# Visual-Behavior/detr-tensorflow

Hardware: AMD Instinct MI355X
Metric: images/sec training step, DETR-R50 800x1333 bs=8/GPU (higher is better)
Workload: dtype bf16

## Files before the change

detr-tensorflow_amd/csrc/optim.hip:

```cpp
#include "common.h"

namespace detr {

__global__ __launch_bounds__(256) void sumsq_segments_kernel(const float *__restrict__ g,
                                                             const int *__restrict__ chunk_tensor,
                                                             const long long *__restrict__ chunk_start,
                                                             const long long *__restrict__ seg_end, int chunk,
                                                             float *__restrict__ sumsq) {
    __shared__ float red[4];
    const int c = blockIdx.x;
    const int t = chunk_tensor[c];
    const long long s0 = chunk_start[c];
    long long s1 = s0 + chunk;
    if (s1 > seg_end[t]) s1 = seg_end[t];
    float acc = 0.f;
    for (long long i = s0 + threadIdx.x; i < s1; i += blockDim.x) {
        const float v = g[i];
        acc += v * v;
    }
    acc = wave_sum(acc);
    if ((threadIdx.x & 63) == 0) red[threadIdx.x >> 6] = acc;
    __syncthreads();
    if (threadIdx.x == 0) sumsq[c] = (red[0] + red[1]) + (red[2] + red[3]);
}

__device__ __forceinline__ float clip_factor(float nrm, float clip) { return nrm > clip ? clip / nrm : (nrm == nrm ? 1.0f : nrm); }

__global__ __launch_bounds__(256) void clip_adam_kernel(float *__restrict__ param, const float *__restrict__ g,
                                                        float *__restrict__ m, float *__restrict__ v,
                                                        const int *__restrict__ chunk_tensor,
                                                        const long long *__restrict__ chunk_start,
                                                        const long long *__restrict__ seg_end,
                                                        const int *__restrict__ tensor_group,
                                                        const float *__restrict__ sumsq,
                                                        const float *__restrict__ hyper, int chunk, int n_chunks) {
    const int c = blockIdx.x;
    const int t = chunk_tensor[c];
    const long long s0 = chunk_start[c];
    long long s1 = s0 + chunk;
    if (s1 > seg_end[t]) s1 = seg_end[t];
    const int grp = tensor_group[t];
    if (grp < 0) return;
    const float lr_t = hyper[grp];
    const float clip = hyper[3], b1 = hyper[4], b2 = hyper[5], eps = hyper[6];
    float cs = 1.0f;
    if (clip > 0.f) {
        __shared__ int s_lo, s_hi;
        __shared__ float s_red[4];
        if (threadIdx.x == 0) {
            int a = 0, b = c;
            while (a < b) { const int mid = (a + b) >> 1; if (chunk_tensor[mid] < t) a = mid + 1; else b = mid; }
            s_lo = a;
            a = c; b = n_chunks;
            while (a < b) { const int mid = (a + b) >> 1; if (chunk_tensor[mid] <= t) a = mid + 1; else b = mid; }
            s_hi = a;
        }
        __syncthreads();
        float acc = 0.f;
        for (int k = s_lo + (int)threadIdx.x; k < s_hi; k += blockDim.x) acc += sumsq[k];
        acc = wave_sum(acc);
        if ((threadIdx.x & 63) == 0) s_red[threadIdx.x >> 6] = acc;
        __syncthreads();
        const float nrm = sqrtf((s_red[0] + s_red[1]) + (s_red[2] + s_red[3]));
        cs = clip_factor(nrm, clip);
    }
    for (long long i = s0 + threadIdx.x; i < s1; i += blockDim.x) {
        const float gi = g[i] * cs;
        const float mi = b1 * m[i] + (1.0f - b1) * gi;
        const float vi = b2 * v[i] + (1.0f - b2) * gi * gi;
        m[i] = mi;
        v[i] = vi;
        param[i] = param[i] - lr_t * mi / (sqrtf(vi) + eps);
    }
}

__global__ void set_floats8_kernel(float *dst, float v0, float v1, float v2, float v3, float v4, float v5, float v6,
                                   float v7) {
    if (threadIdx.x == 0 && blockIdx.x == 0) {
        dst[0] = v0; dst[1] = v1; dst[2] = v2; dst[3] = v3; dst[4] = v4; dst[5] = v5; dst[6] = v6; dst[7] = v7;
    }
}

struct Floats16 { float v[16]; };

__global__ void set_floats16_kernel(float *dst, Floats16 f) {
    if (blockIdx.x == 0 && threadIdx.x < 16) dst[threadIdx.x] = f.v[threadIdx.x];
}

__global__ __launch_bounds__(256) void global_clip_scale_kernel(const float *__restrict__ sumsq,
                                                                const int *__restrict__ chunk_tensor,
                                                                const int *__restrict__ tensor_group,
                                                                const float *__restrict__ hyper, int n_chunks,
                                                                float *__restrict__ scale) {
    __shared__ float red[4];
    float acc = 0.f;
    for (int k = threadIdx.x; k < n_chunks; k += 256) {
        const int grp = tensor_group[chunk_tensor[k]];
        if (grp >= 0 && hyper[11 + grp] != 0.f) acc += sumsq[k];
    }
    acc = wave_sum(acc);
    if ((threadIdx.x & 63) == 0) red[threadIdx.x >> 6] = acc;
// ... 252 lines not shown
```

detr-tensorflow_amd/csrc/rowops.hip:

```cpp
#include "common.h"

namespace detr {

constexpr int LN_MAXV = 4;

__device__ __forceinline__ unsigned ln_pk_bf16(float a, float b) {
    typedef __bf16 bf16x2_t __attribute__((ext_vector_type(2)));
    bf16x2_t r;
    r[0] = (__bf16)a;
    r[1] = (__bf16)b;
    return __builtin_bit_cast(unsigned, r);
}

__global__ __launch_bounds__(256) void layernorm_fwd_kernel(const float *__restrict__ x, const float *__restrict__ gamma,
                                                            const float *__restrict__ beta, float *__restrict__ y,
                                                            float *__restrict__ mean, float *__restrict__ rstd,
                                                            int rows, int C, float eps, const float *__restrict__ add,
                                                            int add_rows, float *__restrict__ y2, unsigned short *__restrict__ y16) {
    const int lane = threadIdx.x & 63;
    const int wpb = blockDim.x >> 6;
    const int nv = C >> 2;
    for (int row = blockIdx.x * wpb + (threadIdx.x >> 6); row < rows; row += gridDim.x * wpb) {
        const float4 *xr = reinterpret_cast<const float4 *>(x + (long long)row * C);
        float4 v[LN_MAXV];
// ... 319 lines not shown
                           C, d->dgamma, d->dbeta);
        DETR_LAUNCH_CHECK("layernorm bwd finish");
    }
    return 0;
}

namespace detr {
typedef __bf16 bf16x2_t __attribute__((ext_vector_type(2)));
__device__ __forceinline__ unsigned pk2_bf16(float a, float b) {
    bf16x2_t r;
    r[0] = (__bf16)a;
    r[1] = (__bf16)b;
    return __builtin_bit_cast(unsigned, r);
}
__global__ void cvt_bf16_kernel(const float4 *__restrict__ x, uint2 *__restrict__ out, long long n4) {
    for (long long i = blockIdx.x * (long long)blockDim.x + threadIdx.x; i < n4; i += (long long)gridDim.x * blockDim.x) {
        const float4 v = x[i];
        out[i] = make_uint2(pk2_bf16(v.x, v.y), pk2_bf16(v.z, v.w));
    }
}
__global__ void scale_cols_bf16_kernel(const float4 *__restrict__ w, const float4 *__restrict__ scale, uint2 *__restrict__ out,
                                       long long n4, int c4) {
    for (long long i = blockIdx.x * (long long)blockDim.x + threadIdx.x; i < n4; i += (long long)gridDim.x * blockDim.x) {
        const float4 v = w[i], sc = scale[i % c4];
        out[i] = make_uint2(pk2_bf16(v.x * sc.x, v.y * sc.y), pk2_bf16(v.z * sc.z, v.w * sc.w));
    }
}

static_assert(sizeof(detr_scale_entry) == 40, "detr_scale_entry layout changed: update Engine._refold_group");

__global__ void scale_cols_bf16_group_kernel(const detr_scale_entry *__restrict__ tab) {
    const detr_scale_entry e = tab[blockIdx.y];
    const float4 *w = reinterpret_cast<const float4 *>(e.w), *scale = reinterpret_cast<const float4 *>(e.scale);
    uint2 *out = reinterpret_cast<uint2 *>(e.out);
    for (long long i = blockIdx.x * (long long)blockDim.x + threadIdx.x; i < e.n4; i += (long long)gridDim.x * blockDim.x) {
        const float4 v = w[i], sc = scale[i % e.c4];
        out[i] = make_uint2(pk2_bf16(v.x * sc.x, v.y * sc.y), pk2_bf16(v.z * sc.z, v.w * sc.w));
    }
}
}

extern "C" int detr_hip_scale_cols_bf16_group(const detr_scale_entry *table, int32_t n, void *stream) {
    DETR_REQUIRE(table && n > 0 && n <= 65535, "scale_cols_bf16_group: bad args");
    hipLaunchKernelGGL(scale_cols_bf16_group_kernel, dim3(64, (unsigned)n), dim3(256), 0, (hipStream_t)stream, table);
    DETR_LAUNCH_CHECK("scale_cols_bf16_group");
    return 0;
}

extern "C" int detr_hip_cvt_bf16(const float *x, uint16_t *out, int64_t n, void *stream) {
    DETR_REQUIRE(x && out && n > 0 && n % 4 == 0 && aligned16(x) && ((uintptr_t)out % 8 == 0), "cvt_bf16: bad args");
    const long long n4 = n / 4;
    long long grid = (n4 + 255) / 256;
    if (grid > 8192) grid = 8192;
    hipLaunchKernelGGL(cvt_bf16_kernel, dim3((unsigned)grid), dim3(256), 0, (hipStream_t)stream, (const float4 *)x, (uint2 *)out, n4);
    DETR_LAUNCH_CHECK("cvt_bf16");
    return 0;
}

extern "C" int detr_hip_scale_cols_bf16(const float *w, const float *scale, uint16_t *out, int64_t rows, int32_t cols,
                                        void *stream) {
    DETR_REQUIRE(w && scale && out && rows > 0 && cols > 0 && cols % 4 == 0, "scale_cols_bf16: bad args");
    DETR_REQUIRE(aligned16(w) && aligned16(scale) && ((uintptr_t)out % 8 == 0), "scale_cols_bf16: alignment");
    const long long n4 = rows * (long long)(cols / 4);
    long long grid = (n4 + 255) / 256;
    if (grid > 8192) grid = 8192;
    hipLaunchKernelGGL(scale_cols_bf16_kernel, dim3((unsigned)grid), dim3(256), 0, (hipStream_t)stream, (const float4 *)w,
                       (const float4 *)scale, (uint2 *)out, n4, cols / 4);
    DETR_LAUNCH_CHECK("scale_cols_bf16");
    return 0;
}

extern "C" int detr_hip_colsum_f32(const float *x, float *out, int64_t rows, int32_t cols, int64_t ld, float alpha,
                                   void *stream) {
    DETR_REQUIRE(x && out && rows > 0 && cols > 0, "colsum: bad args");
    int rpb = 64;
    while ((rows + rpb - 1) / rpb > 2048) rpb *= 2;
    dim3 grid((unsigned)cdiv(cols, 256), (unsigned)((rows + rpb - 1) / rpb));
    hipLaunchKernelGGL(colsum_kernel, grid, dim3(256), 0, (hipStream_t)stream, x, out, (long long)rows, cols,
                       (long long)ld, alpha, rpb);
    DETR_LAUNCH_CHECK("colsum");
    return 0;
}

__global__ __launch_bounds__(256) void colsum_partial_kernel(const float *__restrict__ x, float *__restrict__ part, long long rows, int cols,
                                                             long long ld, int rows_per_block) {
    const int c = blockIdx.x * 256 + threadIdx.x;
    if (c >= cols) return;
    const long long r0 = (long long)blockIdx.y * rows_per_block;
    const long long r1 = (r0 + rows_per_block < rows) ? r0 + rows_per_block : rows;
    float s0 = 0.f, s1 = 0.f;
    long long r = r0;
    for (; r + 1 < r1; r += 2) {
        s0 += x[r * ld + c];
        s1 += x[(r + 1) * ld + c];
    }
    if (r < r1) s0 += x[r * ld + c];
    part[(long long)blockIdx.y * cols + c] = s0 + s1;
}
__global__ __launch_bounds__(256) void colsum_finish_kernel(const float *__restrict__ part, float *__restrict__ out, int chunks, int cols, float alpha) {
    const int c = blockIdx.x * 256 + threadIdx.x;
    if (c >= cols) return;
    float s = 0.f;
    for (int k = 0; k < chunks; ++k) s += part[(long long)k * cols + c];
    out[c] += alpha * s;
}
static int colsum_det_rpb(int64_t rows) {
    int rpb = 64;
    while ((rows + rpb - 1) / rpb > 256) rpb *= 2;
    return rpb;
}
extern "C" int64_t detr_hip_colsum_det_scratch_floats(int64_t rows, int32_t cols) {
    if (rows <= 0 || cols <= 0) return -1;
    const int rpb = colsum_det_rpb(rows);
    return ((rows + rpb - 1) / rpb) * (int64_t)cols;
}
extern "C" int detr_hip_colsum_det_f32(const float *x, float *out, int64_t rows, int32_t cols, int64_t ld, float alpha, float *scratch,
                                       int64_t scratch_floats, void *stream) {
    DETR_REQUIRE(x && out && scratch && rows > 0 && cols > 0, "colsum_det: bad args");
    const int rpb = colsum_det_rpb(rows);
    const int chunks = (int)((rows + rpb - 1) / rpb);
    DETR_REQUIRE(scratch_floats >= (int64_t)chunks * cols, "colsum_det: scratch holds %lld floats, %lld needed", (long long)scratch_floats,
                 (long long)chunks * cols);
    hipLaunchKernelGGL(colsum_partial_kernel, dim3((unsigned)cdiv(cols, 256), (unsigned)chunks), dim3(256), 0, (hipStream_t)stream, x, scratch,
                       (long long)rows, cols, (long long)ld, rpb);
    hipLaunchKernelGGL(colsum_finish_kernel, dim3((unsigned)cdiv(cols, 256)), dim3(256), 0, (hipStream_t)stream, scratch, out, chunks, cols, alpha);
    DETR_LAUNCH_CHECK("colsum_det");
    return 0;
}

extern "C" int detr_hip_add_bcast_f32(const float *x, const float *p, float *out, int64_t n, int64_t period,
                                      void *stream) {
    DETR_REQUIRE(x && p && out && n > 0 && period > 0, "add_bcast: bad args");
    DETR_REQUIRE(n % 4 == 0 && period % 4 == 0 && aligned16(x) && aligned16(p) && aligned16(out), "add_bcast: alignment");
    hipLaunchKernelGGL(add_bcast_kernel, dim3(capped_grid(n / 4, 256, 8192)), dim3(256), 0, (hipStream_t)stream, (const float4 *)x,
                       (const float4 *)p, (float4 *)out, (long long)(n / 4), (long long)(period / 4));
    DETR_LAUNCH_CHECK("add_bcast");
    return 0;
}

extern "C" int detr_hip_add_f32(const float *a, const float *b, float *out, int64_t n, void *stream) {
    DETR_REQUIRE(a && b && out && n > 0, "add: bad args");
    hipLaunchKernelGGL(add_kernel, dim3(capped_grid(n, 256, 8192)), dim3(256), 0, (hipStream_t)stream, a, b, out, (long long)n);
    DETR_LAUNCH_CHECK("add");
    return 0;
}

extern "C" int detr_hip_sigmoid_bwd_f32(const float *dy, const float *y, float *dz, int64_t n, void *stream) {
    DETR_REQUIRE(dy && y && dz && n > 0, "sigmoid_bwd: bad args");
    hipLaunchKernelGGL(sigmoid_bwd_kernel, dim3(capped_grid(n, 256, 8192)), dim3(256), 0, (hipStream_t)stream, dy, y, dz,
                       (long long)n);
    DETR_LAUNCH_CHECK("sigmoid_bwd");
    return 0;
}

extern "C" int detr_hip_dropout_f32(const float *x, float *out, int64_t n, float p, uint32_t site, const uint32_t *step,
                                    void *stream) {
    DETR_REQUIRE(x && out && n > 0 && p >= 0.0f && p < 1.0f, "dropout: bad args");
    hipLaunchKernelGGL(dropout_kernel, dim3(capped_grid(n, 256, 8192)), dim3(256), 0, (hipStream_t)stream, x, out, (long long)n,
                       1.0f / (1.0f - p), drop_thresh16(p), site, step);
    DETR_LAUNCH_CHECK("dropout");
    return 0;
}

namespace detr {
__global__ __launch_bounds__(256) void multi_copy_kernel(const detr_copy_entry *__restrict__ table) {
    const detr_copy_entry e = table[blockIdx.y];
    const uint4 *src = reinterpret_cast<const uint4 *>(e.src);
    uint4 *dst = reinterpret_cast<uint4 *>(e.dst);
    for (long long i = blockIdx.x * (long long)blockDim.x + threadIdx.x; i < e.n16; i += (long long)gridDim.x * blockDim.x) {
        if (e.mode == 0) {
            dst[i] = src[i];
        } else {
            const float4 a = reinterpret_cast<const float4 *>(src)[i];
            float4 b = reinterpret_cast<float4 *>(dst)[i];
            b.x += a.x; b.y += a.y; b.z += a.z; b.w += a.w;
            reinterpret_cast<float4 *>(dst)[i] = b;
        }
    }
}
__global__ void set_u32x8_kernel(uint32_t *dst, uint32_t v0, uint32_t v1, uint32_t v2, uint32_t v3, uint32_t v4, uint32_t v5,
                                 uint32_t v6, uint32_t v7) {
    if (threadIdx.x == 0) { dst[0] = v0; dst[1] = v1; dst[2] = v2; dst[3] = v3; dst[4] = v4; dst[5] = v5; dst[6] = v6; dst[7] = v7; }
}
}

namespace detr {
// ... 98 lines not shown
```

detr-tensorflow_amd/csrc/setloss.hip:

```cpp
#include "common.h"
#include <limits.h>
#include <cmath>
#include <type_traits>

namespace detr {

struct SetLossArgs {
    int levels, B, Q, C, R;
    const float *logits; long long sL_l, sL_b, sL_q;
    const float *boxes;  long long sB_l, sB_b, sB_q;
    const float *t_bbox; const long long *t_class;
    int background_class;
};

struct FixedCriterion {
    static constexpr float cost_class = 1.0f, cost_bbox = 5.0f, cost_giou = 2.0f;
    static constexpr float w_label = 1.0f, w_bbox = 5.0f, w_giou = 2.0f;
    static constexpr float eos = 0.1f;
    static constexpr bool weighted = false;
    __device__ __forceinline__ float class_weight(int, int) const { return 1.0f; }
    __device__ __forceinline__ float weight_sum(const float *s) const { return eos * s[3] + s[4]; }
    __device__ __forceinline__ float box_count(float npos) const { return npos; }
};

// ... 154 lines not shown

constexpr int SL_QCHUNK = 8;

template <class Crit, class Cls>
__global__ __launch_bounds__(256) void match_cost_kernel(SetLossArgs a, Crit crit, Cls clsterm, float *__restrict__ cost) {
    __shared__ typename Cls::Row s_row[SL_QCHUNK];
    __shared__ float s_t[SL_MAXR][4];
    __shared__ int s_cls[SL_MAXR];
    const int p = blockIdx.x;
    const int lv = p / a.B, b = p % a.B;
    const int n = header_n(a.t_bbox, b, a.R);
    const int ldc = a.R - 1;
    if (n == 0) return;
    const float *lg = a.logits + lv * a.sL_l + b * a.sL_b;
    const float *bx = a.boxes + lv * a.sB_l + b * a.sB_b;
    const int lane = threadIdx.x & 63, wave = threadIdx.x >> 6;
    for (int j = threadIdx.x; j < n; j += blockDim.x) {
        const float *t = a.t_bbox + ((long long)b * a.R + 1 + j) * 4;
        s_t[j][0] = t[0]; s_t[j][1] = t[1]; s_t[j][2] = t[2]; s_t[j][3] = t[3];
        s_cls[j] = (int)a.t_class[(long long)b * a.R + 1 + j];
    }
    const int q0 = blockIdx.y * SL_QCHUNK, q1 = min(a.Q, q0 + SL_QCHUNK);
    for (int q = q0 + wave; q < q1; q += 4) {
        const typename Cls::Row r = clsterm.row_stats(lg + q * a.sL_q, a.C, lane);
        if (lane == 0) s_row[q - q0] = r;
    }
    __syncthreads();
    float *out = cost + (long long)p * a.Q * ldc;
    for (int idx = threadIdx.x; idx < (q1 - q0) * n; idx += blockDim.x) {
        const int ql = idx / n, j = idx - ql * n;
        const int q = q0 + ql;
        const float *pb = bx + q * a.sB_q;
        const float pcx = pb[0], pcy = pb[1], pw = pb[2], ph = pb[3];
        const float tcx = s_t[j][0], tcy = s_t[j][1], tw = s_t[j][2], th = s_t[j][3];
        const int cls = s_cls[j];
        const float cost_class = (cls >= 0 && cls < a.C) ? clsterm.cost(s_row[ql], lg[q * a.sL_q + cls]) : 0.0f;
        const float cost_bbox = fabsf(pcx - tcx) + fabsf(pcy - tcy) + fabsf(pw - tw) + fabsf(ph - th);
        const float cost_giou = -giou_of(to_xyxy(pcx, pcy, pw, ph), to_xyxy(tcx, tcy, tw, th));
        out[q * ldc + j] = crit.cost_bbox * cost_bbox + crit.cost_class * cost_class + crit.cost_giou * cost_giou;
    }
}

template <int CTRL, int ROW_MASK>
__device__ __forceinline__ double dpp_min_step(double x, int &tlo, int &thi) {
    tlo = __builtin_amdgcn_update_dpp(tlo, __double2loint(x), CTRL, ROW_MASK, 0xf, false);
    thi = __builtin_amdgcn_update_dpp(thi, __double2hiint(x), CTRL, ROW_MASK, 0xf, false);
    const double y = __hiloint2double(thi, tlo);
    double r;
    asm("v_min_f64 %0, %1, %2" : "=v"(r) : "v"(x), "v"(y));
    return r;
}
__device__ __forceinline__ double wave_min_f64_dpp(double x) {
    int tlo = __double2loint(x), thi = __double2hiint(x);
    x = dpp_min_step<0x111, 0xf>(x, tlo, thi);
    x = dpp_min_step<0x112, 0xf>(x, tlo, thi);
    x = dpp_min_step<0x114, 0xf>(x, tlo, thi);
    x = dpp_min_step<0x118, 0xf>(x, tlo, thi);
    x = dpp_min_step<0x142, 0xa>(x, tlo, thi);
    x = dpp_min_step<0x143, 0xc>(x, tlo, thi);
    const int lo = __builtin_amdgcn_readlane(__double2loint(x), 63);
    const int hi = __builtin_amdgcn_readlane(__double2hiint(x), 63);
    return __hiloint2double(hi, lo);
}

template <int S, int N>
struct AssignPick {
    static __device__ __forceinline__ void run(unsigned long long (&todo)[N], unsigned long long (&live)[N],
                                               const unsigned long long (&freecol)[N], const int (&row4col)[N], int &jstar,
                                               int &r4, bool &isfree) {
        if (S + 1 == N || todo[S]) {
            const int l = ((int)__ffsll((long long)todo[S]) - 1) & 63;
            const unsigned long long bit = 1ull << l;
            todo[S] &= ~bit;
            live[S] &= ~bit;
            isfree = (freecol[S] & bit) != 0ull;
            r4 = __builtin_amdgcn_readlane(row4col[S], l);
            jstar = 64 * S + l;
        } else {
            AssignPick<(S + 1 < N ? S + 1 : S), N>::run(todo, live, freecol, row4col, jstar, r4, isfree);
        }
    }
};

template <int MAXCPL, bool CD>
__global__ __launch_bounds__(64) void assign_kernel(const float *__restrict__ cost, int Q, int ldc,
                                                    const float *__restrict__ t_bbox, int B, int R,
                                                    int *__restrict__ tgt_for_pred, int *__restrict__ pred_for_tgt,
                                                    int *__restrict__ status) {
    using CT = typename std::conditional<CD, double, float>::type;
    extern __shared__ __attribute__((aligned(16))) char smem[];
    const int p = blockIdx.x, b = p % B, lane = threadIdx.x;
    const int nmax = (R + 1) & ~1;
    const int n = header_n(t_bbox, b, R);
    const int cpl = (Q + 63) >> 6;
    const int Qs = CD ? MAXCPL * 64 + 1 : cpl * 64 + 1;
    double *u0 = reinterpret_cast<double *>(smem);
    int *col4row = reinterpret_cast<int *>(u0 + nmax);
    CT *cT = reinterpret_cast<CT *>(col4row + nmax);
    double *u = CD ? reinterpret_cast<double *>(cT) + (Qs - 1) : u0;
    const int us = CD ? Qs : 1;

    for (int q = lane; q < Q; q += 64) tgt_for_pred[(long long)p * Q + q] = -1;
    for (int j = lane; j < ldc; j += 64) pred_for_tgt[(long long)p * ldc + j] = -1;
    if (lane == 0) status[p] = 0;
    if (n == 0) return;
    if (n > Q) {
        if (lane == 0) status[p] = 2;
        return;
    }
    const float *Cg = cost + (long long)p * Q * ldc;
    bool bad = false;
    for (int idx = lane; idx < Q * n; idx += 64) {
        const int q = idx / n, j = idx - q * n;
        const float c = Cg[q * ldc + j];
        cT[j * Qs + q] = (CT)c;
        bad |= !(c == c) || (c == -INFINITY);
    }
    if (Qs > Q)
        for (int idx = lane; idx < (Qs - Q) * n; idx += 64) cT[(idx / (Qs - Q)) * Qs + Q + idx % (Qs - Q)] = (CT)INFINITY;
    __syncthreads();
    for (int i = lane; i < n; i += 64) {
        u[i * us] = 0.0;
        col4row[i] = -1;
    }
    __syncthreads();
    if (__any(bad)) {
        if (lane == 0) status[p] = 1;
        return;
    }
    double v[MAXCPL], spc[MAXCPL];
    int path[MAXCPL], row4col[MAXCPL];
    unsigned long long exist[MAXCPL];
    unsigned long long freecol[MAXCPL];
#pragma unroll
    for (int s = 0; s < MAXCPL; ++s) {
        v[s] = 0.0;
        spc[s] = INFINITY;
        path[s] = -1;
        row4col[s] = -1;
        const int cnt = Q - 64 * s;
        exist[s] = cnt >= 64 ? ~0ull : (cnt <= 0 ? 0ull : ((1ull << cnt) - 1ull));
        freecol[s] = exist[s];
    }
    for (int i = 0; i < n; ++i) {
        const CT *crow = cT + i * Qs;
        double best = INFINITY;
        int bestj = INT_MAX;
#pragma unroll
        for (int s = 0; s < MAXCPL; ++s) {
            const int j = lane + 64 * s;
            if (s < cpl && j < Q) {
                const double c = (double)crow[j];
                if (c < best) { best = c; bestj = j; }
            }
        }
        const double gmin = wave_min_f64_dpp(best);
        if (!(gmin < (double)INFINITY)) continue;
        const unsigned long long mall = __ballot(best == gmin);
        const int ownl = __ffsll((long long)mall) - 1;
        const int jstar = __builtin_amdgcn_readlane(bestj, ownl);
        const int owns = jstar >> 6;
        int r4 = -1;
#pragma unroll
        for (int s = 0; s < MAXCPL; ++s)
            if (s == owns) r4 = row4col[s];
        r4 = __builtin_amdgcn_readlane(r4, ownl);
        if (lane == 0) u[i * us] = gmin;
        if (r4 == -1) {
#pragma unroll
            for (int s = 0; s < MAXCPL; ++s) {
                if (s == owns && lane == ownl) row4col[s] = i;
                if (s == owns) freecol[s] &= ~(1ull << ownl);
            }
            if (lane == 0) col4row[i] = jstar;
        }
    }
    __syncthreads();
    bool infeasible = false;
    for (int cur = 0; cur < n; ++cur) {
        if (col4row[cur] != -1) continue;
        double minVal = 0.0;
        int i = cur;
        int sink = -1;
        unsigned long long live[MAXCPL], todo[MAXCPL];
#pragma unroll
        for (int s = 0; s < MAXCPL; ++s) {
            spc[s] = INFINITY;
            live[s] = exist[s];
            todo[s] = 0ull;
        }
        while (true) {
            const double ui = u[i * us];
            const CT *crow = cT + i * Qs + lane;
            CT cf[MAXCPL];
#pragma unroll
            for (int s = 0; s < MAXCPL; ++s) cf[s] = crow[CD ? 64 * s : 64 * (s < cpl ? s : cpl - 1)];
            unsigned long long any_todo = 0ull;
#pragma unroll
            for (int s = 0; s < MAXCPL; ++s) {
                const double r = minVal + (double)cf[s] - ui - v[s];
                const unsigned long long um = __builtin_amdgcn_ballot_w64(r < spc[s]) & live[s];
                const bool upd = __builtin_amdgcn_inverse_ballot_w64(um);
// ... 434 lines not shown
```

detr-tensorflow_amd/detr_tf/engine.py:

```python
import math
import os
from ctypes import byref, c_float
from typing import NamedTuple, Optional

import numpy as np
import torch

from . import _hip as hip
from .params import ParamStore, RESNET50_BLOCKS, block_names, bn_conv_pairs, stem_names
from .streams import DropMasks, SideStream

D = 256
HEADS = 8
HD = 32
FF = 2048
BN_EPS = 1e-5
KERAS_BN_EPS = 1.001e-5
LN_EPS = 1e-5
DEFER_REDUCE = os.environ.get("DETR_HIP_DEFER_REDUCE", "1") != "0"
WGRAD_STREAM = os.environ.get("DETR_HIP_WGRAD_STREAM", "1") != "0"
BWD_FUSED = os.environ.get("DETR_HIP_BWD_FUSED", "1") != "0"
DROPMASK_AHEAD = int(os.environ.get("DETR_HIP_DROPMASK_AHEAD", "2") or 0)
QK_ALPHA = float(HD) ** -0.5 * 1.4426950408889634


def mix32(x):
    x &= 0xFFFFFFFF
    x ^= x >> 16
    x = (x * 0x7FEB352D) & 0xFFFFFFFF
    x ^= x >> 15
    x = (x * 0x846CA68B) & 0xFFFFFFFF
    x ^= x >> 16
    return x


def step_seed(base_seed, step_no, rank=0):
    return mix32(mix32((base_seed + 0x9E3779B9 * step_no) & 0xFFFFFFFF) ^ ((rank * 0x85EBCA6B) & 0xFFFFFFFF))


def position_embedding_sine_host(H, W, num_pos_features=128, temperature=10000.0, eps=1e-6):
    y = (np.arange(1, H + 1, dtype=np.float32) / np.float32(H + eps) * np.float32(2 * math.pi)).astype(np.float32)
    x = (np.arange(1, W + 1, dtype=np.float32) / np.float32(W + eps) * np.float32(2 * math.pi)).astype(np.float32)
    k = np.arange(num_pos_features, dtype=np.float32)
    dim_t = np.power(np.float32(temperature), (2 * np.floor(k / 2) / np.float32(num_pos_features)).astype(np.float32)).astype(np.float32)
    py = (y[:, None] / dim_t[None, :]).astype(np.float32)
    px = (x[:, None] / dim_t[None, :]).astype(np.float32)
    ey = np.empty_like(py)
    ex = np.empty_like(px)
    ey[:, 0::2], ey[:, 1::2] = np.sin(py[:, 0::2]), np.cos(py[:, 1::2])
    ex[:, 0::2], ex[:, 1::2] = np.sin(px[:, 0::2]), np.cos(px[:, 1::2])
    pos = np.concatenate([np.broadcast_to(ey[:, None, :], (H, W, num_pos_features)),
                          np.broadcast_to(ex[None, :, :], (H, W, num_pos_features))], axis=2)
    return np.ascontiguousarray(pos.reshape(H * W, 2 * num_pos_features), dtype=np.float32)


def position_embedding_sine_table(n_max, num_pos_features=128, temperature=10000.0, eps=1e-6):
    k = np.arange(num_pos_features, dtype=np.float32)
    dim_t = np.power(np.float32(temperature), (2 * np.floor(k / 2) / np.float32(num_pos_features)).astype(np.float32)).astype(np.float32)
    tab = np.zeros((n_max + 1, n_max + 1, num_pos_features), np.float32)
    c = np.arange(0, n_max + 1, dtype=np.float32)
    for n in range(n_max + 1):
        y = (c / np.float32(n + eps) * np.float32(2 * math.pi)).astype(np.float32)
        py = (y[:, None] / dim_t[None, :]).astype(np.float32)
        tab[n, :, 0::2], tab[n, :, 1::2] = np.sin(py[:, 0::2]), np.cos(py[:, 1::2])
    return tab


def downsample_mask_nearest(mask, Hf, Wf):
    mask = np.asarray(mask)
    H, W = mask.shape[1:]
    sy = np.minimum((np.arange(Hf) * H) // Hf, H - 1)
    sx = np.minimum((np.arange(Wf) * W) // Wf, W - 1)
    return mask[:, sy][:, :, sx]


def dilation_flags(replace_stride_with_dilation):
    if replace_stride_with_dilation is None:
        return (False, False, False)
    flags = tuple(bool(f) for f in replace_stride_with_dilation)
    if len(flags) != 3:
        raise ValueError(f"replace_stride_with_dilation: expected 3 flags (layer2, layer3, layer4), got {len(flags)}")
    return flags


def feature_size(H, W, replace_stride_with_dilation=None):
    for halves in (True, True) + tuple(not f for f in dilation_flags(replace_stride_with_dilation)):
        if halves:
            H, W = (H - 1) // 2 + 1, (W - 1) // 2 + 1
    return H, W


def backbone_stride(replace_stride_with_dilation=None):
    return 4 * 2 ** sum(1 for f in dilation_flags(replace_stride_with_dilation) if not f)


class Block(NamedTuple):
    p: str
    n: dict
    x: torch.Tensor
    xs: torch.Tensor
    x1: torch.Tensor
    y1: torch.Tensor
    y2: torch.Tensor
    out: torch.Tensor
    h: int
    w: int
    ho: int
    wo: int
    h1: int
    w1: int
    M1: int
    s2: int
    cin: int
    d1: int
    d2: int
    stride: int
    first: bool
    out_bits: Optional[torch.Tensor]
    dil: int


class DetrEngine:
    def __init__(self, device="cuda:0", blocks=RESNET50_BLOCKS, num_enc=6, num_dec=6, num_queries=100,
                 num_classes=92, nb_class=None, seed=0, tf_backbone=False, replace_stride_with_dilation=(False, False, False)):
        self.dilate = dilation_flags(replace_stride_with_dilation)
        if tf_backbone and any(self.dilate):
            raise ValueError("replace_stride_with_dilation needs the reference backbone: tf.keras.applications.ResNet50 "
                             "(tf_backbone=True) has no such option")
        hip.load()
        self.device = torch.device(device)
        hip.ensure_workspace(self.device)
        if DEFER_REDUCE:
            hip.ensure_defer_workspace(self.device)
        self.blocks = tuple(blocks)
        self.num_enc, self.num_dec, self.Q = num_enc, num_dec, num_queries
        self.nb_class = nb_class
        self.C = num_classes if nb_class is None else nb_class
        self.tf_backbone = bool(tf_backbone)
        self.bn_eps = KERAS_BN_EPS if self.tf_backbone else BN_EPS
        self.P = ParamStore(self.device, blocks, num_enc, num_dec, num_queries, num_classes, nb_class, seed, tf_backbone=tf_backbone)
        self._stem = stem_names(self.tf_backbone)
        self._pairs = bn_conv_pairs(self.blocks, self.tf_backbone)
        self._bufs = {}
        self._buf_gen = 0
        self._pos_cache = {}
        self._pos_tables = {}
        self.key_valid = None
        self._attn_sites = ()
        self.attn_maps = {}
        self._shape = None
        self._adt = torch.float32
        self._block_recs = []
        self._feat_meta = None
        self._fold_table = self._shift_table = None
        self.bn_scale, self.bn_shift = {}, {}
        self._weights_version, self._built = 0, {}
        self.P.on_change = self._params_changed
        self.fold_bn()
        self.compute = 0
        self.f32_split = False
        self.dropout_p = 0.1
        self.dropout_seed = 0x5EED
        self.dp_rank = 0
        self._step_no = 0
        self._drop = (0.0, 0)
        self._step_seed = 0
        self._seed_dev = torch.zeros(8, dtype=torch.int32, device=self.device)
        self._cross = {}
        self._graph_replay = False
        self.phase_events = None
        self.side = SideStream(self.device)
        self.masks = DropMasks(self, HEADS)

    @property
    def gemm_mode(self):
        return 1 if self.compute == 1 else (2 if self.f32_split else 0)

    def bump_weights_version(self):
        self._weights_version += 1

    def _stale(self, key):
        if self._built.get(key) == self._weights_version:
            return False
        self._built[key] = self._weights_version
        return True

    def seed_of_step(self, step_no):
        return step_seed(self.dropout_seed, step_no, self.dp_rank)

    def advance_dropout_step(self):
        self._step_no += 1
        self._step_seed = self.seed_of_step(self._step_no)
        self.masks.settle()
        hip.call("detr_hip_set_u32x8", self._seed_dev.data_ptr(), self._step_seed, self.seed_of_step(self._step_no + 1),
                 0, 0, 0, 0, 0, 0)
        self._drop = (float(self.dropout_p), self._step_seed)
        return self._step_seed

    def phase(self, name):
        if self.phase_events is not None:
            ev = torch.cuda.Event(enable_timing=True)
            ev.record()
            self.phase_events.append((name, ev))

    def buf(self, name, shape, dtype=torch.float32):
        key = name
        t = self._bufs.get(key)
        shape = tuple(int(s) for s in shape)
        if t is None or tuple(t.shape) != shape or t.dtype != dtype:
            if t is not None:
                self._buf_gen += 1
            t = torch.empty(shape, dtype=dtype, device=self.device)
            self._bufs[key] = t
        return t

    @property
    def buf_generation(self):
        return self._buf_gen + hip.WS_GENERATION

    def buffer_bytes(self):
        return sum(t.numel() * t.element_size() for t in self._bufs.values())

    def fold_bn(self):
        for p, c in self.P.bn.items():
            raw = self.P.bn_raw[p]
            sc = self.buf(f"bnscale:{p}", (c,))
            sh = self.buf(f"bnshift:{p}", (c,))
            hip.call("detr_hip_bn_fold_f32", raw[0].data_ptr(), raw[1].data_ptr(), raw[2].data_ptr(), raw[3].data_ptr(),
                     sc.data_ptr(), sh.data_ptr(), c, c_float(self.bn_eps))
            self.bn_scale[p] = sc
            self.bn_shift[p] = self.buf(f"bnshift_eff:{p}", (c,)) if self.tf_backbone else sh
        self.bump_weights_version()
        self._fold_table = None
        self._shift_table = None

    def _refresh_bias_shift(self):
        if self._shift_table is None:
            rows = []
            for bn_name, conv_name in self._pairs:
                c = self.P.bn[bn_name]
                rows.append([self.P.views[f"{conv_name}/bias"].data_ptr(), self.bn_scale[bn_name].data_ptr(),
                             self._bufs[f"bnshift:{bn_name}"].data_ptr(), self.bn_shift[bn_name].data_ptr(), c])
            self._shift_table = torch.tensor(rows, dtype=torch.int64).to(self.device)
        hip.call("detr_hip_fma_vec_group", self._shift_table.data_ptr(), self._shift_table.shape[0])

    def _params_changed(self):
        self.fold_bn()

    def load_params(self, params):
        return self.P.load_dict(params)

    def _w(self, name):
        if self.compute == 1 and self.P.views16 is not None:
            return self.P.views16[name]
        return self.P.views[name]

    def _refresh_shadow(self):
        flat16 = self.P.shadow16()
        hip.call("detr_hip_cvt_bf16", self.P.flat.data_ptr(), flat16.data_ptr(), self.P.flat.numel())
        self._refold_group()

    def _refold_group(self):
        if self._fold_table is None:
            rows = []
            for bn_name, conv in self._pairs[1:]:
                conv_name = f"{conv}/kernel"
                w = self.P.views[conv_name]
                co = w.shape[-1]
                ws16 = self.buf(f"ws16:{conv_name}", w.shape, torch.bfloat16)
                rows.append([w.data_ptr(), self.bn_scale[bn_name].data_ptr(), ws16.data_ptr(), w.numel() // 4, co // 4])
            self._fold_table = torch.tensor(rows, dtype=torch.int64).to(self.device)
            self._fold_keep = [self.bn_scale, self._bufs]
        hip.call("detr_hip_scale_cols_bf16_group", self._fold_table.data_ptr(), self._fold_table.shape[0])

    def _scaled_kernel(self, conv_name, bn_name):
        w = self.P.views[conv_name]
        co = w.shape[-1]
        if self.compute == 1 and conv_name != f"{self._stem['conv']}/kernel":
            return self.buf(f"ws16:{conv_name}", w.shape, torch.bfloat16)
        ws = self.buf(f"ws:{conv_name}", w.shape)
        if self._stale(f"ws:{conv_name}"):
            hip.call("detr_hip_scale_cols_f32", w.data_ptr(), self.bn_scale[bn_name].data_ptr(), ws.data_ptr(),
                     w.numel() // co, co)
        return ws

    def _conv1x1_fwd(self, x, M, cin, cout, conv_name, bn_name, out, residual=None, act=1, maskbits_out=None):
        ws = self._scaled_kernel(conv_name, bn_name)
        shift = self.bn_shift[bn_name]
        ldr = cout if residual is not None else 0
        hip.gemm(M, cout, cin, x, cin, 1, ws, cout, 0, out, cout, bias=shift, residual=residual, ldr=ldr, act=act,
                 maskbits_out=maskbits_out)

    @staticmethod
    def _wgrad(M_out, N_out, K_red, A, lda, Bm, ldb, C, ldc, scale=None, alpha=1.0, compute=None):
        args, kwargs = hip.wgrad_call(M_out, N_out, K_red, A, lda, Bm, ldb, C, ldc, scale=scale, alpha=alpha, compute=compute)
        hip.gemm(*args, **kwargs)

    def _a16(self, base):
        return (f"{base}16", torch.bfloat16) if self.compute == 1 else (base, torch.float32)

    def _colsum(self, x2d, out, alpha=1.0):
        rows, cols = x2d.shape
        n = int(hip.load().detr_hip_colsum_det_scratch_floats(rows, cols))
        scratch = self.buf(f"colsum:{rows}x{cols}", (n,))
        hip.call("detr_hip_colsum_det_f32", x2d.data_ptr(), out.data_ptr(), rows, cols, x2d.stride(0), c_float(alpha),
                 scratch.data_ptr(), n)

    def _ln_fwd(self, x, pfx, y, tag, add=None, y2=None, y16=None):
        rows = x.shape[0]
        mean = self.buf(f"{tag}:mean", (rows,))
        rstd = self.buf(f"{tag}:rstd", (rows,))
        hip.layernorm_fwd(x, self.P.views[f"{pfx}/gamma"], self.P.views[f"{pfx}/beta"], y, mean, rstd, LN_EPS, add=add, y2=y2,
                          y16=y16)

    def _ln_spec(self, rows, pfx, y, tag, add=None, y2=None, y16=None, ffn=False):
        if self.compute != 1 or ffn:
            return None
        return dict(gamma=self.P.views[f"{pfx}/gamma"], beta=self.P.views[f"{pfx}/beta"], y=y, mean=self.buf(f"{tag}:mean", (rows,)),
                    rstd=self.buf(f"{tag}:rstd", (rows,)), eps=LN_EPS, add=add, y2=y2, y16=y16)

    def _ln_bwd(self, dy, x, pfx, dx, tag, dx_add=None, drop_site=None, want16=False, dy_add=None):
        dp, _ = self._drop
        dx_drop = dx_drop16 = None
        if drop_site is not None:
            if want16:
                dx_drop16 = self.buf(f"scratch:drop16:{dx.shape[0]}{self.side.suffix(tag)}", dx.shape, torch.bfloat16)
            elif dp > 0.0:
                dx_drop = self.buf(f"scratch:drop:{dx.shape[0]}{self.side.suffix(tag)}", dx.shape)
        hip.layernorm_bwd(dy, x, self.P.views[f"{pfx}/gamma"], self._bufs[f"{tag}:mean"], self._bufs[f"{tag}:rstd"], dx,
                          self.P.gviews[f"{pfx}/gamma"], self.P.gviews[f"{pfx}/beta"], dx_add=dx_add, dx_drop=dx_drop,
                          dropout_p=dp, dropout_site=(drop_site or 0), dropout_step=self._seed_dev, dx_drop16=dx_drop16,
                          dy_add=dy_add)
        if dx_drop16 is not None:
            return dx_drop16
        return dx if dx_drop is None else dx_drop

    def _add_bcast(self, x, p, out):
        hip.call("detr_hip_add_bcast_f32", x.data_ptr(), p.data_ptr(), out.data_ptr(), x.numel(), p.numel())

    @property
    def attn16(self):
        return self.compute == 1

    def pregen_dropmasks_at_matcher(self):
        self.masks.at_matcher()

    def _self_attn_fwd(self, tag, pfx, qk_in, v_in, B, T, out, site, ln=None, key_valid=None):
        W, bias = self._w(f"{pfx}/in_proj_kernel"), self.P.views[f"{pfx}/in_proj_bias"]
        dp, _ = self._drop
        lse = self.buf(f"{tag}:lse", (B * HEADS, T))
        if self.attn16:
            QKV = self.buf(f"{tag}:QKV16", (B * T, 3 * D), torch.bfloat16)
            hip.gemm_group([hip.linear_fwd_call(qk_in, W[0:D], bias[0:D], QKV[:, 0:D], alpha=QK_ALPHA),
# ... 689 lines not shown
```

detr-tensorflow_amd/detr_tf/params.py:

```python
import math
from collections import OrderedDict

import numpy as np
import torch

RESNET50_BLOCKS = (3, 4, 6, 3)
RESNET101_BLOCKS = (3, 4, 23, 3)
GROUPS = ("backbone", "transformers", "nlayers")


def variable_group(name, nlayers):
    top = name.split("/", 1)[0]
    if top in nlayers:
        return 2
    if top == "transformer" or top.startswith("class_embed") or top.startswith("bbox_embed"):
        return 1
    return 0


def block_names(li, b, tf_backbone=False):
    if tf_backbone:
        q = f"resnet50/conv{li + 2}_block{b + 1}"
        return dict(conv1=f"{q}_1_conv", bn1=f"{q}_1_bn", conv2=f"{q}_2_conv", bn2=f"{q}_2_bn", conv3=f"{q}_3_conv", bn3=f"{q}_3_bn",
                    down=f"{q}_0_conv", bnd=f"{q}_0_bn", tag=f"{q}")
# ... 57 lines not shown
        ln(f"{p}/norm2")
    s["input_proj/kernel"] = (1, 1, 2048, model_dim)
    s["input_proj/bias"] = (model_dim,)
    s["query_embed/kernel"] = (num_queries, model_dim)
    cins = [64]
    for li in range(4):
        cins.append(256 * 2 ** li)
    def conv(name, shape):
        s[f"{name}/kernel"] = shape
        if tf_backbone:
            s[f"{name}/bias"] = (shape[3],)

    for li in reversed(range(4)):
        d1 = 64 * 2 ** li
        d2 = 4 * d1
        for b in reversed(range(blocks[li])):
            cin = cins[li] if b == 0 else d2
            n = block_names(li, b, tf_backbone)
            conv(n["conv3"], (1, 1, d1, d2))
            conv(n["conv2"], (3, 3, d1, d1))
            conv(n["conv1"], (1, 1, cin, d1))
            if b == 0:
                conv(n["down"], (1, 1, cin, d2))
    conv(stem_names(tf_backbone)["conv"], (7, 7, 3, 64))
    return s


def bn_names(blocks, tf_backbone=False):
    out = OrderedDict()
    out[stem_names(tf_backbone)["bn"]] = 64
    for li in range(4):
        d1 = 64 * 2 ** li
        d2 = 4 * d1
        for b in range(blocks[li]):
            n = block_names(li, b, tf_backbone)
            out[n["bn1"]] = d1
            out[n["bn2"]] = d1
            out[n["bn3"]] = d2
            if b == 0:
                out[n["bnd"]] = d2
    return out


def bn_conv_pairs(blocks, tf_backbone=False):
    st = stem_names(tf_backbone)
    out = [(st["bn"], st["conv"])]
    for li in range(4):
        for b in range(blocks[li]):
            n = block_names(li, b, tf_backbone)
            out += [(n["bn1"], n["conv1"]), (n["bn2"], n["conv2"]), (n["bn3"], n["conv3"])]
            if b == 0:
                out.append((n["bnd"], n["down"]))
    return out


class ParamStore:
    def __init__(self, device, blocks=RESNET50_BLOCKS, num_enc=6, num_dec=6, num_queries=100, num_classes=92,
                 nb_class=None, seed=0, tf_backbone=False):
        self.device = device
        self.tf_backbone = bool(tf_backbone)
        self.blocks = tuple(blocks)
        self.bn_leaves = BN_LEAVES[self.tf_backbone]
        self.shapes = trainable_shapes(blocks, num_enc, num_dec, num_queries, num_classes, nb_class, tf_backbone=tf_backbone)
        self.bn = bn_names(blocks, tf_backbone)
        self.offsets = OrderedDict()
        off = 0
        for k, shp in self.shapes.items():
            n = int(np.prod(shp))
            self.offsets[k] = (off, n)
            off += (n + 7) // 8 * 8
        self.total = off
        self.flat = torch.zeros(self.total, dtype=torch.float32, device=device)
        self.grad = torch.zeros(self.total, dtype=torch.float32, device=device)
        self.views = {k: self.flat[o:o + n].view(self.shapes[k]) for k, (o, n) in self.offsets.items()}
        self.gviews = {k: self.grad[o:o + n].view(self.shapes[k]) for k, (o, n) in self.offsets.items()}
        self.flat16, self.views16 = None, None
        self.on_change = None
        self.ema, self.ema_num_updates, self.ema_swapped = None, 0, False
        self.bn_raw = {p: torch.zeros(4, c, dtype=torch.float32, device=device) for p, c in self.bn.items()}
        for p in self.bn_raw:
            self.bn_raw[p][3].fill_(1.0)
        self.init_random(seed)

    def shadow16(self):
        if self.flat16 is None:
            self.flat16 = torch.zeros(self.total, dtype=torch.bfloat16, device=self.device)
            self.views16 = {k: self.flat16[o:o + n].view(self.shapes[k]) for k, (o, n) in self.offsets.items()}
        return self.flat16

    def init_random(self, seed):
        rng = np.random.default_rng(seed)
        host = np.zeros(self.total, np.float32)
        for k, shp in self.shapes.items():
            o, n = self.offsets[k]
            if len(shp) == 4:
                fan_in, fan_out = shp[0] * shp[1] * shp[2], shp[0] * shp[1] * shp[3]
            elif len(shp) == 2:
                fan_in, fan_out = shp[1], shp[0]
            else:
                fan_in = fan_out = shp[0]
            if k.endswith("gamma"):
                v = np.ones(shp, np.float32)
            elif k.endswith("beta"):
                v = np.zeros(shp, np.float32)
            else:
                lim = math.sqrt(6.0 / (fan_in + fan_out))
                v = rng.uniform(-lim, lim, shp).astype(np.float32)
            host[o:o + n] = v.ravel()
        self.flat.copy_(torch.from_numpy(host))
        for p, c in self.bn.items():
            lim = math.sqrt(6.0 / (2 * c))
            raw = np.stack([rng.uniform(-lim, lim, c), rng.uniform(-lim, lim, c), np.zeros(c), np.ones(c)]).astype(np.float32)
            self.bn_raw[p].copy_(torch.from_numpy(raw))

    def load_dict(self, params):
        if self.ema_swapped:
            raise RuntimeError("load_weights: not inside ema_weights(model) -- the parameter buffer holds the averaged weights there")
        missing = []
        staged = []
        for k in self.shapes:
            if k in params:
                v = torch.as_tensor(np.asarray(params[k]), dtype=torch.float32)
                if tuple(v.shape) != tuple(self.shapes[k]):
                    raise ValueError(f"{k}: shape {tuple(v.shape)} != {self.shapes[k]}")
                staged.append((self.views[k], v))
            else:
                missing.append(k)
        for p in self.bn:
            for i, leaf in enumerate(self.bn_leaves):
                if f"{p}/{leaf}" in params:
                    v = torch.as_tensor(np.asarray(params[f"{p}/{leaf}"]), dtype=torch.float32)
                    if v.numel() != self.bn_raw[p][i].numel():
                        raise ValueError(f"{p}/{leaf}: {v.numel()} values != {self.bn_raw[p][i].numel()}")
                    staged.append((self.bn_raw[p][i], v.reshape(self.bn_raw[p][i].shape)))
                else:
                    missing.append(f"{p}/{leaf}")
        try:
            for dst, v in staged:
                dst.copy_(v)
            self.reset_ema()
        finally:
            if self.on_change is not None:
                self.on_change()
        return missing

    def reset_ema(self):
        if self.ema is not None:
            self.ema.copy_(self.flat)
            self.ema_num_updates = 0

    def state_dict(self, weights="model"):
        if weights not in ("model", "ema"):
            raise ValueError(f"weights must be 'model' or 'ema', got {weights!r}")
        if weights == "ema":
            if self.ema is None:
                raise ValueError("weights='ema': this model has no averaged weights (config.ema_decay was never set)")
            host = (self.flat if self.ema_swapped else self.ema).cpu().numpy()
            out = {k: host[o:o + n].reshape(self.shapes[k]).copy() for k, (o, n) in self.offsets.items()}
        else:
            out = {k: v.detach().cpu().numpy().copy() for k, v in self.views.items()}
        for p in self.bn:
            for i, leaf in enumerate(self.bn_leaves):
                out[f"{p}/{leaf}"] = self.bn_raw[p][i].cpu().numpy().copy()
        return out

    def save(self, path, weights="model"):
        np.savez(path, **self.state_dict(weights))

    def load(self, path):
        with np.load(path) as z:
            return self.load_dict({k: z[k] for k in z.files})
# ... 30 lines not shown
```

Measured before the change: 532.7.

## Batch loads in reductions and assign staging; skip redundant bf16 shadow of folded convs

The gradient sum-of-squares, column-sum and assignment-cost staging kernels now issue batches of independent loads before consuming them, so more memory requests are in flight per thread. The bf16 parameter shadow refresh no longer converts the whole flat buffer. Conv kernels that are already BN-folded into separate bf16 buffers are skipped, and the remaining ranges become extra rows of the existing grouped scale_cols launch. This removes one full-buffer conversion kernel and its traffic, at the cost of more fold-table rows and a new env switch to restore the old path.

```diff
diff --git a/detr-tensorflow_amd/csrc/optim.hip b/detr-tensorflow_amd/csrc/optim.hip
--- a/detr-tensorflow_amd/csrc/optim.hip
+++ b/detr-tensorflow_amd/csrc/optim.hip
@@ -1,6 +1,8 @@
 #include "common.h"
 
 namespace detr {
+
+constexpr int SUMSQ_BATCH = 16;
 
 __global__ __launch_bounds__(256) void sumsq_segments_kernel(const float *__restrict__ g,
                                                              const int *__restrict__ chunk_tensor,
@@ -14,9 +16,18 @@
     long long s1 = s0 + chunk;
     if (s1 > seg_end[t]) s1 = seg_end[t];
     float acc = 0.f;
-    for (long long i = s0 + threadIdx.x; i < s1; i += blockDim.x) {
-        const float v = g[i];
-        acc += v * v;
+    for (long long b0 = s0; b0 < s1; b0 += (long long)SUMSQ_BATCH * 256) {
+        const float *gb = g + b0 + threadIdx.x;
+        float v[SUMSQ_BATCH];
+        if (b0 + (long long)SUMSQ_BATCH * 256 <= s1) {
+#pragma unroll
+            for (int k = 0; k < SUMSQ_BATCH; ++k) v[k] = gb[k * 256];
+        } else {
+#pragma unroll
+            for (int k = 0; k < SUMSQ_BATCH; ++k) v[k] = b0 + threadIdx.x + k * 256 < s1 ? gb[k * 256] : 0.f;
+        }
+#pragma unroll
+        for (int k = 0; k < SUMSQ_BATCH; ++k) acc = __fmaf_rn(v[k], v[k], acc);
     }
     acc = wave_sum(acc);
     if ((threadIdx.x & 63) == 0) red[threadIdx.x >> 6] = acc;
diff --git a/detr-tensorflow_amd/csrc/rowops.hip b/detr-tensorflow_amd/csrc/rowops.hip
--- a/detr-tensorflow_amd/csrc/rowops.hip
+++ b/detr-tensorflow_amd/csrc/rowops.hip
@@ -425,6 +425,7 @@
     return 0;
 }
 
+constexpr int COLSUM_BATCH = 16;
 __global__ __launch_bounds__(256) void colsum_partial_kernel(const float *__restrict__ x, float *__restrict__ part, long long rows, int cols,
                                                              long long ld, int rows_per_block) {
     const int c = blockIdx.x * 256 + threadIdx.x;
@@ -432,19 +433,30 @@
     const long long r0 = (long long)blockIdx.y * rows_per_block;
     const long long r1 = (r0 + rows_per_block < rows) ? r0 + rows_per_block : rows;
     float s0 = 0.f, s1 = 0.f;
-    long long r = r0;
-    for (; r + 1 < r1; r += 2) {
-        s0 += x[r * ld + c];
-        s1 += x[(r + 1) * ld + c];
-    }
-    if (r < r1) s0 += x[r * ld + c];
+    for (long long r = r0; r < r1; r += COLSUM_BATCH) {
+        float v[COLSUM_BATCH];
+#pragma unroll
+        for (int j = 0; j < COLSUM_BATCH; ++j) v[j] = x[(r + j < r1 ? r + j : r1 - 1) * ld + c];
+#pragma unroll
+        for (int j = 0; j < COLSUM_BATCH; j += 2) {
+            if (r + j < r1) s0 += v[j];
+            if (r + j + 1 < r1) s1 += v[j + 1];
+        }
+    }
     part[(long long)blockIdx.y * cols + c] = s0 + s1;
 }
 __global__ __launch_bounds__(256) void colsum_finish_kernel(const float *__restrict__ part, float *__restrict__ out, int chunks, int cols, float alpha) {
     const int c = blockIdx.x * 256 + threadIdx.x;
     if (c >= cols) return;
     float s = 0.f;
-    for (int k = 0; k < chunks; ++k) s += part[(long long)k * cols + c];
+    for (int k = 0; k < chunks; k += COLSUM_BATCH) {
+        float v[COLSUM_BATCH];
+#pragma unroll
+        for (int j = 0; j < COLSUM_BATCH; ++j) v[j] = part[(long long)(k + j < chunks ? k + j : chunks - 1) * cols + c];
+#pragma unroll
+        for (int j = 0; j < COLSUM_BATCH; ++j)
+            if (k + j < chunks) s += v[j];
+    }
     out[c] += alpha * s;
 }
 static int colsum_det_rpb(int64_t rows) {
diff --git a/detr-tensorflow_amd/csrc/setloss.hip b/detr-tensorflow_amd/csrc/setloss.hip
--- a/detr-tensorflow_amd/csrc/setloss.hip
+++ b/detr-tensorflow_amd/csrc/setloss.hip
@@ -260,6 +260,21 @@
     }
 };
 
+constexpr int ASSIGN_STAGE_BATCH = 8;
+
+struct TileWalk {
+    int r, c, dr, dc, w;
+    __device__ __forceinline__ TileWalk(int lane, int w_) : r(lane / w_), c(lane % w_), dr(64 / w_), dc(64 % w_), w(w_) {}
+    __device__ __forceinline__ void next() {
+        r += dr;
+        c += dc;
+        if (c >= w) {
+            c -= w;
+            ++r;
+        }
+    }
+};
+
 template <int MAXCPL, bool CD>
 __global__ __launch_bounds__(64) void assign_kernel(const float *__restrict__ cost, int Q, int ldc,
                                                     const float *__restrict__ t_bbox, int B, int R,
@@ -288,14 +303,36 @@
     }
     const float *Cg = cost + (long long)p * Q * ldc;
     bool bad = false;
-    for (int idx = lane; idx < Q * n; idx += 64) {
-        const int q = idx / n, j = idx - q * n;
-        const float c = Cg[q * ldc + j];
-        cT[j * Qs + q] = (CT)c;
-        bad |= !(c == c) || (c == -INFINITY);
-    }
-    if (Qs > Q)
-        for (int idx = lane; idx < (Qs - Q) * n; idx += 64) cT[(idx / (Qs - Q)) * Qs + Q + idx % (Qs - Q)] = (CT)INFINITY;
+    const int total = Q * n;
+    TileWalk wk(lane, n);
+    for (int idx0 = lane; idx0 < total; idx0 += 64 * ASSIGN_STAGE_BATCH) {
+        float c[ASSIGN_STAGE_BATCH];
+        int slot[ASSIGN_STAGE_BATCH];
+#pragma unroll
+        for (int k = 0; k < ASSIGN_STAGE_BATCH; ++k) {
+            const bool ok = idx0 + 64 * k < total;
+            c[k] = Cg[ok ? wk.r * ldc + wk.c : 0];
+            slot[k] = ok ? wk.c * Qs + wk.r : -1;
+            wk.next();
+        }
+        static_assert(ASSIGN_STAGE_BATCH == 8, "list every staged value here");
+        asm volatile("" : "+v"(c[0]), "+v"(c[1]), "+v"(c[2]), "+v"(c[3]), "+v"(c[4]), "+v"(c[5]), "+v"(c[6]), "+v"(c[7]));
+#pragma unroll
+        for (int k = 0; k < ASSIGN_STAGE_BATCH; ++k) {
+            if (slot[k] >= 0) {
+                cT[slot[k]] = (CT)c[k];
+                bad |= !(c[k] == c[k]) || (c[k] == -INFINITY);
+            }
+        }
+    }
+    if (Qs > Q) {
+        const int w = Qs - Q;
+        TileWalk pw(lane, w);
+        for (int idx = lane; idx < w * n; idx += 64) {
+            cT[pw.r * Qs + Q + pw.c] = (CT)INFINITY;
+            pw.next();
+        }
+    }
     __syncthreads();
     for (int i = lane; i < n; i += 64) {
         u[i * us] = 0.0;
diff --git a/detr-tensorflow_amd/detr_tf/engine.py b/detr-tensorflow_amd/detr_tf/engine.py
--- a/detr-tensorflow_amd/detr_tf/engine.py
+++ b/detr-tensorflow_amd/detr_tf/engine.py
@@ -21,6 +21,8 @@
 WGRAD_STREAM = os.environ.get("DETR_HIP_WGRAD_STREAM", "1") != "0"
 BWD_FUSED = os.environ.get("DETR_HIP_BWD_FUSED", "1") != "0"
 DROPMASK_AHEAD = int(os.environ.get("DETR_HIP_DROPMASK_AHEAD", "2") or 0)
+SHADOW_FULL = os.environ.get("DETR_HIP_SHADOW_FULL", "0") == "1"
+SHADOW_PIECE = 64 * 256 * 8 * 4
 QK_ALPHA = float(HD) ** -0.5 * 1.4426950408889634
 
 
@@ -153,6 +155,7 @@
         self._block_recs = []
         self._feat_meta = None
         self._fold_table = self._shift_table = None
+        self.shadow_full = SHADOW_FULL
         self.bn_scale, self.bn_shift = {}, {}
         self._weights_version, self._built = 0, {}
         self.P.on_change = self._params_changed
@@ -255,9 +258,15 @@
             return self.P.views16[name]
         return self.P.views[name]
 
+    def _shadow_skip(self):
+        if self.shadow_full:
+            return frozenset()
+        return frozenset(f"{conv}/kernel" for _, conv in self._pairs[1:])
+
     def _refresh_shadow(self):
-        flat16 = self.P.shadow16()
-        hip.call("detr_hip_cvt_bf16", self.P.flat.data_ptr(), flat16.data_ptr(), self.P.flat.numel())
+        flat16 = self.P.shadow16(skip=self._shadow_skip())
+        if self.shadow_full:
+            hip.call("detr_hip_cvt_bf16", self.P.flat.data_ptr(), flat16.data_ptr(), self.P.flat.numel())
         self._refold_group()
 
     def _refold_group(self):
@@ -269,6 +278,14 @@
                 co = w.shape[-1]
                 ws16 = self.buf(f"ws16:{conv_name}", w.shape, torch.bfloat16)
                 rows.append([w.data_ptr(), self.bn_scale[bn_name].data_ptr(), ws16.data_ptr(), w.numel() // 4, co // 4])
+            if not self.shadow_full:
+                ones = self.buf("shadow_unit_scale", (4,))
+                ones.fill_(1.0)
+                src, dst = self.P.flat.data_ptr(), self.P.flat16.data_ptr()
+                for lo, hi in self.P.shadow_ranges(self._shadow_skip()):
+                    for a in range(lo, hi, SHADOW_PIECE):
+                        n = min(SHADOW_PIECE, hi - a)
+                        rows.append([src + 4 * a, ones.data_ptr(), dst + 2 * a, n // 4, 1])
             self._fold_table = torch.tensor(rows, dtype=torch.int64).to(self.device)
             self._fold_keep = [self.bn_scale, self._bufs]
         hip.call("detr_hip_scale_cols_bf16_group", self._fold_table.data_ptr(), self._fold_table.shape[0])
diff --git a/detr-tensorflow_amd/detr_tf/params.py b/detr-tensorflow_amd/detr_tf/params.py
--- a/detr-tensorflow_amd/detr_tf/params.py
+++ b/detr-tensorflow_amd/detr_tf/params.py
@@ -163,11 +163,25 @@
             self.bn_raw[p][3].fill_(1.0)
         self.init_random(seed)
 
-    def shadow16(self):
+    def shadow16(self, skip=()):
         if self.flat16 is None:
             self.flat16 = torch.zeros(self.total, dtype=torch.bfloat16, device=self.device)
-            self.views16 = {k: self.flat16[o:o + n].view(self.shapes[k]) for k, (o, n) in self.offsets.items()}
+            self.views16 = {k: self.flat16[o:o + n].view(self.shapes[k]) for k, (o, n) in self.offsets.items() if k not in skip}
         return self.flat16
+
+    def shadow_ranges(self, skip=()):
+        names = list(self.offsets)
+        out = []
+        for i, k in enumerate(names):
+            if k in skip:
+                continue
+            lo = self.offsets[k][0]
+            hi = self.offsets[names[i + 1]][0] if i + 1 < len(names) else self.total
+            if out and out[-1][1] == lo:
+                out[-1] = (out[-1][0], hi)
+            else:
+                out.append((lo, hi))
+        return out
 
     def init_random(self, seed):
         rng = np.random.default_rng(seed)
```

After: 536.1, median of 6. No clear change (+0.6%).
